# ultravideo/video-stitcher

Hardware: AMD Instinct MI355X
Metric: stitched frames/sec, 6x1080p->4K equirect (ms/frame = 1000/value*n_gpus) (higher is better)
Workload: dtype u8 in / int16+fp32 pyramid arithmetic; 1 GPU; cfg2: 6x1920x1080 views -> 3840x1920 equirect, spherical, 5 bands, CPW off; a step = 20 passes over a batch of 96 frames per GPU (1920 frames), each pass on 3 HIP stream(s) / contexts, inputs resident in HBM; distinct_frame_sets=8, frames_per_pass=96, streams=3, parallelism=frame-parallel x1

## Files before the change

video-stitcher_amd/csrc/compositor.hip:

```cpp
#include <algorithm>
#include <climits>
#include <memory>
#include <mutex>
#include <new>
#include <vector>
#include "common.hpp"
#include "launchers.hpp"
#include "descs.hpp"
#include "ctx.hpp"

namespace ms {

__device__ __forceinline__ void sample3(const uint8_t *__restrict__ src, unsigned sstep, int srows, int scols,
                                        float xc, float yc, float out[3])
{
    const int x1 = f2i_rd(xc), y1 = f2i_rd(yc);
    const int x2 = (int)((unsigned)x1 + 1u), y2 = (int)((unsigned)y1 + 1u);
    const float wx2 = (float)x2 - xc, wx1 = xc - (float)x1;
    const float wy2 = (float)y2 - yc, wy1 = yc - (float)y1;
    const float w[4] = {wx2 * wy2, wx1 * wy2, wx2 * wy1, wx1 * wy1};
    const int xs[4] = {x1, x2, x1, x2};
    const int ys[4] = {y1, y1, y2, y2};
    out[0] = out[1] = out[2] = 0.f;
#pragma unroll
    for (int t = 0; t < 4; ++t) {
        const bool inb = xs[t] >= 0 && xs[t] < scols && ys[t] >= 0 && ys[t] < srows;
        const uint8_t *p = src + (size_t)(inb ? ys[t] : 0) * sstep + (size_t)(inb ? xs[t] : 0) * 3;
#pragma unroll
        for (int c = 0; c < 3; ++c) out[c] = __builtin_fmaf(inb ? (float)p[c] : 0.f, w[t], out[c]);
    }
}

// ... 798 lines not shown
                } else {
                    const int k0 = (q >> 1) * 4 + (q & 1), k1 = k0 + 2;
                    DivBy d0(1.f), d1(1.f);
                    d0.d = den[r][k0]; d0.r = rcp[r][k0]; d1.d = den[r][k1]; d1.r = rcp[r][k1];
                    const int n0 = trunc_s16(d0((float)(int)(int16_t)(a & 0xffffu))), n1 = trunc_s16(d1((float)((int)a >> 16)));
                    n = ((unsigned)n0 & 0xffffu) | ((unsigned)n1 << 16);
                }
                resq[c][r][q] = addsat_pk_i16(upq[r][q], n);
            }
    }

    if (!L0) {
        const size_t plane = (size_t)P.qh[l] * P.qpitch[l];
        int16_t *d = cl + (size_t)f * cl_stride + P.coff[l] + (mul24(y0, P.qpitch[l]) + (unsigned)x0);
#pragma unroll
        for (int c = 0; c < 3; ++c)
#pragma unroll
            for (int r = 0; r < 2; ++r) {
                uint4 o;
                o.x = __builtin_amdgcn_perm(resq[c][r][1], resq[c][r][0], 0x05040100u);
                o.y = __builtin_amdgcn_perm(resq[c][r][1], resq[c][r][0], 0x07060302u);
                o.z = __builtin_amdgcn_perm(resq[c][r][3], resq[c][r][2], 0x05040100u);
                o.w = __builtin_amdgcn_perm(resq[c][r][3], resq[c][r][2], 0x07060302u);
                *reinterpret_cast<uint4 *>(d + c * plane + (size_t)r * P.qpitch[l]) = o;
            }
    } else {
#pragma unroll
        for (int r = 0; r < 2; ++r) {
            const int y = y0 + r;
            if (y >= P.fh) continue;
            const uint8_t *mrow = P.mask + mul24(y, P.mask_pitch);
            const int nvalid = min(8, P.fw - x0);
            uint2 mk8 = make_uint2(0u, 0u);
            if (nvalid == 8) __builtin_memcpy(&mk8, __builtin_assume_aligned(mrow + x0, 8), 8);
            else {
#pragma unroll
                for (int k = 0; k < 8; ++k) {
                    const unsigned m = (k < nvalid) ? (unsigned)mrow[x0 + k] : 0u;
                    if (k < 4) mk8.x |= m << (8 * k); else mk8.y |= m << (8 * (k - 4));
                }
            }
            const unsigned mq[4] = {__builtin_amdgcn_perm(0u, mk8.x, 0x02020000u), __builtin_amdgcn_perm(0u, mk8.x, 0x03030101u),
                                    __builtin_amdgcn_perm(0u, mk8.y, 0x02020000u), __builtin_amdgcn_perm(0u, mk8.y, 0x03030101u)};
            unsigned v[3][4];
#pragma unroll
            for (int c = 0; c < 3; ++c)
#pragma unroll
                for (int q = 0; q < 4; ++q) v[c][q] = resq[c][r][q] & mq[q];
            auto val = [&](int k, int c) -> int {
                const unsigned w = v[c][(k >> 2) * 2 + (k & 1)];
                return ((k >> 1) & 1) ? ((int)w >> 16) : (int)(int16_t)(w & 0xffffu);
            };
            if (out.p16[f]) {
                int16_t *d = (int16_t *)((char *)out.p16[f] + mul24(y, (int)out.step16[f])) + 3 * x0;
                if (nvalid == 8) {
                    unsigned wds[12];
#pragma unroll
// ... 492 lines not shown
            if (l >= 1) {
                const LevelDesc &F = V.lv[l - 1];
                Bits u = dilate(half(Wn[v][l - 1], F.w, F.h), L.w, L.h, 1);
                for (size_t i = 0; i < n.size(); ++i) n[i] |= u[i];
            }
            if (l < nb) {
                const LevelDesc &C = V.lv[l + 1];
                Bits d = dilate(twice(Nd[v][l + 1], C.w, C.h, L.w, L.h), L.w, L.h, 2);
                for (size_t i = 0; i < n.size(); ++i) n[i] |= d[i];
            }
            Nd[v][l] = std::move(n);
        }
        tot0 += (double)V.pw * V.ph;
    }
    c->warp_tiled = true;
    for (int v = 0; v < N; ++v) c->warp_tiled = c->warp_tiled && (c->h_views[v].pw % 4 == 0);
    c->warp_tiled = c->warp_tiled && c->cfg.src_width >= 3 && c->cfg.src_height >= 2;
    for (int v = 0; v < N; ++v) c->warp_tiled = c->warp_tiled && c->h_views[v].aw >= 3 && c->h_views[v].ah >= 2;
    {
        std::vector<WarpTile> tiles;
        for (int v = 0; v < N; ++v) {
            if (!((c->own_mask >> v) & 1u)) continue;
            const ViewDesc &V = c->h_views[v];
            for (int y0 = 0; y0 < V.ph; y0 += WARP_TH)
                for (int x0 = 0; x0 < V.pw; x0 += WARP_TW)
                    if (any_in(Nd[v][0], V.pw, V.ph, x0, y0, WARP_TW, WARP_TH)) {
                        WarpTile t{};
                        t.view = (short)v; t.x0 = (short)x0; t.y0 = (short)y0;
                        if (!c->custom_maps && x0 >= V.left && x0 + WARP_TW <= V.left + V.aw && y0 >= V.top && y0 + WARP_TH <= V.top + V.ah) {
                            t.flags |= 4;
                            t.ctab = (int)(c->tab_off[v] + (size_t)(x0 - V.left));
                            t.rtab = (int)(c->tab_off[v] + (size_t)round_up(V.aw, 4) + (size_t)(y0 - V.top));
                        }
                        tiles.push_back(t);
                        need0 += (double)std::min(WARP_TW, V.pw - x0) * std::min(WARP_TH, V.ph - y0);
                    }
        }
        c->needed_mask = 0;
        for (const WarpTile &t : tiles) c->needed_mask |= 1u << t.view;
        for (int v = 0; v < MAX_VIEWS; ++v) c->warp_per_view[v] = 0;
        for (const WarpTile &t : tiles) ++c->warp_per_view[t.view];
        if (!windowed || !c->warp_tiled) c->needed_mask = 0xffffffffu;
        if (c->cfg.raster_tile_order == 0) xcd_order(tiles, dev_knob("MS_XCD_CHUNK_WARP", c->cfg.enable_cpw ? 0 : 32));
        c->n_warp_tiles = (int)tiles.size();
        if (int e = c->warp_tiles.alloc(std::max<size_t>(1, tiles.size()) * sizeof(WarpTile))) return e;
        c->warp_lds_tiles = 0;
        if (!tiles.empty()) {
            MS_HIP(hipMemcpy(c->warp_tiles.p, tiles.data(), tiles.size() * sizeof(WarpTile), hipMemcpyHostToDevice));
            if (c->warp_tiled) {
                k_tile_bbox<<<c->n_warp_tiles, dim3(WARP_BX, std::min(WARP_TH, 256 / WARP_BX))>>>((WarpTile *)c->warp_tiles.p, (const ViewDesc *)c->view_tab.p, c->cfg.src_height, c->cfg.src_width, 0);
                MS_LAUNCH_CHECK();
                MS_HIP(hipMemcpy(tiles.data(), c->warp_tiles.p, tiles.size() * sizeof(WarpTile), hipMemcpyDeviceToHost));
                double sw_sum = 0; int sw_n = 0;
                for (const WarpTile &t : tiles) {
                    if (t.flags & 1) ++c->warp_lds_tiles;
                    if (t.sw > 0) { sw_sum += t.sw; ++sw_n; }
                }
                c->warp_minification = sw_n ? sw_sum / sw_n / WARP_TW : 0.0;
// ... 44 lines not shown
            for (const WarpTile &t : tiles) ((t.flags & 2) ? a : b).push_back(t);
            c->n_stage1_reachable = (int)a.size();
            if (c->cfg.raster_tile_order == 0) { xcd_order(a, dev_knob("MS_XCD_CHUNK_S1", 32)); xcd_order(b, dev_knob("MS_XCD_CHUNK_S1", 32)); }
            tiles = a;
            tiles.insert(tiles.end(), b.begin(), b.end());
        }
        c->n_stage1_tiles = (int)tiles.size();
        for (int v = 0; v < MAX_VIEWS; ++v) c->stage1_per_view[v] = 0;
        for (const WarpTile &t : tiles) ++c->stage1_per_view[t.view];
        if (int e = c->stage1_tiles.alloc(std::max<size_t>(1, tiles.size()) * sizeof(WarpTile))) return e;
        MS_HIP(hipMemcpy(c->stage1_tiles.p, tiles.data(), tiles.size() * sizeof(WarpTile), hipMemcpyHostToDevice));
        if (!tiles.empty() && c->warp_tiled) {
            k_tile_bbox<<<c->n_stage1_tiles, dim3(WARP_BX, std::min(WARP_TH, 256 / WARP_BX))>>>((WarpTile *)c->stage1_tiles.p, (const ViewDesc *)c->view_tab.p, c->cfg.src_height, c->cfg.src_width, 1);
            MS_LAUNCH_CHECK();
            MS_HIP(hipDeviceSynchronize());
        }
    }
    for (int l = 0; l < nb; ++l) {
        std::vector<DownTile> tiles;
        if (c->down_vec[l])
            for (int v = 0; v < N; ++v) {
                if (!((c->own_mask >> v) & 1u)) continue;
                const LevelDesc &Lo = c->h_views[v].lv[l + 1];
                for (int y0 = 0; y0 < Lo.h; y0 += DOWN_TH)
                    for (int x0 = 0; x0 < Lo.w; x0 += DOWN_TW)
                        if (any_in(Nd[v][l + 1], Lo.w, Lo.h, x0, y0, DOWN_TW, DOWN_TH)) tiles.push_back(DownTile{(short)v, 0, (short)x0, (short)y0});
            }
        if (c->cfg.raster_tile_order == 0) xcd_order(tiles, dev_knob(l == 0 ? "MS_XCD_CHUNK_DOWN0" : "MS_XCD_CHUNK_DOWN", 0));
        c->n_down_tiles[l] = (int)tiles.size();
        for (int v = 0; v < MAX_VIEWS; ++v) c->down_per_view[l][v] = 0;
        for (const DownTile &t : tiles) ++c->down_per_view[l][t.view];
        if (int e = c->down_tiles[l].alloc(std::max<size_t>(1, tiles.size()) * sizeof(DownTile))) return e;
        if (!tiles.empty()) MS_HIP(hipMemcpy(c->down_tiles[l].p, tiles.data(), tiles.size() * sizeof(DownTile), hipMemcpyHostToDevice));
    }
    for (int l = 0; l < nb; ++l) {
        std::vector<BlendTile> tiles;
        if (c->blend_vec[l])
            for (int y0 = 0; y0 < c->pano.qh[l]; y0 += BLEND_TH)
                for (int x0 = 0; x0 < c->pano.qw[l]; x0 += BLEND_TW) {
                    if (windowed && (x0 + BLEND_TW <= ra[l] || x0 >= rb[l])) continue;
                    unsigned m = 0;
                    for (int v = 0; v < N; ++v) {
                        const LevelDesc &L = c->h_views[v].lv[l];
                        if (any_in(W[v][l], L.w, L.h, x0 - L.x_tl, y0 - L.y_tl, BLEND_TW, BLEND_TH)) m |= 1u << v;
                    }
                    tiles.push_back(BlendTile{(short)x0, (short)y0, m});
                }
        if (c->cfg.raster_tile_order == 0) xcd_order(tiles, dev_knob(l == 0 ? "MS_XCD_CHUNK_BLEND0" : "MS_XCD_CHUNK_BLEND", (l == 0 && c->pano.qw[0] <= 4096) ? 8 : 0));
        c->n_blend_tiles[l] = (int)tiles.size();
// ... 468 lines not shown
}

static const uint8_t *blend_mask_ptr(const ms_ctx *c, int v)
{
    return (c->use_eff[v] ? (const uint8_t *)c->masks_eff.p : (const uint8_t *)c->masks.p) + c->mask_off[v];
}

int ms_init_blender(ms_ctx *c, ms_stream stream)
{
    if (!c) return fail(MS_ERR_INVALID, "null context");
    if (!c->maps_built || !c->masks_built) return fail(MS_ERR_STATE, "ms_init_blender: maps and masks must be built first");
    hipStream_t st = as_stream(stream);
    std::lock_guard<std::recursive_mutex> tables_lk(c->tables_mu);
    if (c->stitch_pending) MS_HIP(hipEventSynchronize(c->last_stitch));
    if (int e = pull_tracked_gains(c)) return e;
    const int nb = c->bg.num_bands, N = c->N, F = c->cfg.max_frames;
    c->act = nullptr; c->subset_on = false;
    ++c->tables_gen;
    if (c->subset_built_set) MS_HIP(hipEventSynchronize(c->subset_built));
    c->subsets.clear();
    c->zero_w.release();

    c->h_views.assign(N, ViewDesc{});
    size_t w_total = 0;
    long long g0_total = 64, gl_total = 64, stage_total = 0;
    c->max_pw = c->max_ph = c->max_aw = c->max_ah = 0;
    for (int v = 0; v < N; ++v) {
        ViewDesc &V = c->h_views[v];
        V.aw = c->roi[v].width; V.ah = c->roi[v].height;
        V.top = c->pad[v].top; V.left = c->pad[v].left;
        V.pw = V.aw + c->pad[v].left + c->pad[v].right;
        V.ph = V.ah + c->pad[v].top + c->pad[v].bottom;
        V.gain = (float)c->gain[v];
        V.xmap = (const float *)c->maps.p + c->map_off[v];
        V.ymap = V.xmap + (size_t)V.ah * c->map_pitch[v];
        V.map_pitch = c->map_pitch[v];
        if (c->custom_maps) V.proj = PROJ_MAPS;
        else {
            V.coltab = (const float2 *)c->tabs.p + c->tab_off[v];
            V.rowtab = V.coltab + round_up(V.aw, 4);
            V.wp = c->wparams[v];
            V.proj = c->cfg.projection;
        }
        V.s1_off = stage_total;
        V.s1_pitch = round_up(V.aw * 3, 4);
        stage_total += (long long)round_up(V.s1_pitch * V.ah + 8, 16);
        c->max_pw = std::max(c->max_pw, V.pw); c->max_ph = std::max(c->max_ph, V.ph);
        c->max_aw = std::max(c->max_aw, V.aw); c->max_ah = std::max(c->max_ah, V.ah);
        int w = V.pw, h = V.ph, xt = c->pad[v].x_tl, yt = c->pad[v].y_tl;
        for (int l = 0; l <= nb; ++l) {
            LevelDesc &L = V.lv[l];
            L.w = w; L.h = h; L.x_tl = xt; L.y_tl = yt;
            L.pitch = round_up(w, 16);
            L.wpitch = round_up(w, 4);
            c->w_off[v][l] = w_total;
            w_total += (size_t)h * L.wpitch;
            if (l == 0) { L.off = g0_total; g0_total += 3LL * h * L.pitch; }
            else        { L.off = gl_total; gl_total += 3LL * h * L.pitch; }
            w = (w + 1) / 2; h = (h + 1) / 2; xt /= 2; yt /= 2;
        }
    }
    for (int l = 0; l < nb; ++l) {
        bool ok = true;
        for (int v = 0; v < N; ++v) {
            const LevelDesc &L = c->h_views[v].lv[l];
            ok = ok && (L.w % 8 == 0) && (L.w >= 8) && (L.h >= 3);
        }
        c->down_vec[l] = ok;
    }
    {
        int t0 = 0;
        while (t0 < nb && c->down_vec[t0]) ++t0;
        auto plan_tail = [&](int l0, int sw, int *out_l0, int *out_lds, int *out_strips) {
            *out_l0 = -1; *out_lds = 0; *out_strips = 1;
            if (l0 < 1 || l0 >= nb) return;
            int need = 0, strips = 1;
            for (int v = 0; v < N; ++v) {
                int w[MAX_LEVELS + 1], a[MAX_LEVELS + 1], b[MAX_LEVELS + 1];
                for (int l = l0; l <= nb; ++l) w[l] = c->h_views[v].lv[l].w;
                const int ns = div_up(w[nb], sw);
                strips = std::max(strips, ns);
                for (int sidx = 0; sidx < ns; ++sidx) {
                    tail_range(w, l0, nb, sidx, sw, a, b);
                    int bytes = 0;
                    for (int l = l0; l <= nb; ++l) bytes += ((b[l] - a[l]) * c->h_views[v].lv[l].h + 15) & ~15;
                    need = std::max(need, bytes);
                }
            }
            if (need <= 64 * 1024) { *out_l0 = l0; *out_lds = need; *out_strips = strips; }
        };
        plan_tail(t0, TAIL_STRIP, &c->tail_l0, &c->tail_lds, &c->tail_strips);
        int l0b = -1;
        plan_tail(t0, TAIL_STRIP_BATCH, &l0b, &c->tail_lds_b, &c->tail_strips_b);
        if (l0b != c->tail_l0) { c->tail_lds_b = c->tail_lds; c->tail_strips_b = c->tail_strips; c->tail_sw_b = TAIL_STRIP; } else c->tail_sw_b = TAIL_STRIP_BATCH;
    }
    for (int l = 0; l < nb; ++l) {
        int qw = c->bg.dst_roi.width >> l, qh = c->bg.dst_roi.height >> l;
        bool ok = (qw % 8 == 0) && (qh % 2 == 0);
        for (int v = 0; v < N; ++v) {
            const LevelDesc &L = c->h_views[v].lv[l];
            ok = ok && (L.w % 8 == 0) && (L.x_tl % 8 == 0) && (L.h % 2 == 0) && (L.y_tl % 2 == 0);
        }
        c->blend_vec[l] = ok;
    }
    c->w_total = w_total;
    if (int e = c->weights.alloc(w_total * sizeof(float))) return e;
    MS_HIP(hipMemsetAsync(c->weights.p, 0, w_total * sizeof(float), st));
    {
        size_t m_total = 0;
        for (int v = 0; v < N; ++v) {
            ViewDesc &V = c->h_views[v];
            V.wm0_pitch = round_up(V.pw, 16);
            c->wm0_off[v] = m_total;
            m_total += (size_t)V.wm0_pitch * V.ph;
        }
        c->wm0_total = m_total + 64;
        if (int e = c->wm0.alloc(m_total + 64)) return e;
        MS_HIP(hipMemsetAsync(c->wm0.p, 0, m_total + 64, st));
        for (int v = 0; v < N; ++v) {
            ViewDesc &V = c->h_views[v];
            V.wm0 = (const uint8_t *)c->wm0.p + c->wm0_off[v];
            MS_HIP(hipMemcpy2DAsync((uint8_t *)c->wm0.p + c->wm0_off[v] + (size_t)V.top * V.wm0_pitch + V.left, V.wm0_pitch,
                                    blend_mask_ptr(c, v), V.aw, V.aw, V.ah, hipMemcpyDeviceToDevice, st));
        }
    }
    for (int v = 0; v < N; ++v)
        for (int l = 0; l <= nb; ++l) c->h_views[v].lv[l].wgt = (const float *)c->weights.p + c->w_off[v][l];

    PanoDesc &P = c->pano;
    P = PanoDesc{};
    P.nb = nb; P.n_views = N;
    size_t den_total = 0;
    long long cl_total = 32, pacc_total = 0;
    {
        int w = c->bg.dst_roi.width, h = c->bg.dst_roi.height;
        for (int l = 0; l <= nb; ++l) {
            P.qw[l] = w; P.qh[l] = h; P.qpitch[l] = round_up(w, 8); P.dpitch[l] = round_up(w, 4);
            c->den_off[l] = den_total; den_total += (size_t)h * P.dpitch[l];
            P.coff[l] = cl_total;
            if (l >= 1) cl_total += 3LL * h * P.qpitch[l];
            P.poff[l] = pacc_total;
            pacc_total += 3LL * h * P.qpitch[l];
            w = (w + 1) / 2; h = (h + 1) / 2;
        }
    }
    P.fw = c->bg.dst_roi_final.width; P.fh = c->bg.dst_roi_final.height;
    P.mask_pitch = round_up(P.fw, 16);
    P.alpha = (float)(1. / 255.);
    P.canvas_x = c->canvas_x; P.canvas_y = c->canvas_y; P.out_w = c->cfg.out_width; P.out_h = c->cfg.out_height;
    P.i_y0 = std::max(0, c->canvas_y & ~1); P.i_rows = std::max(0, std::min(c->cfg.out_height & ~1, (c->canvas_y + P.fh + 1) & ~1) - P.i_y0);
    c->den_total = den_total;
    if (int e = c->den.alloc(den_total * sizeof(float))) return e;
    if (int e = c->result_mask.alloc((size_t)P.mask_pitch * P.fh)) return e;
    MS_HIP(hipMemsetAsync(c->den.p, 0, den_total * sizeof(float), st));
    for (int l = 0; l <= nb; ++l) P.den[l] = (const float *)c->den.p + c->den_off[l];
    P.mask = (const uint8_t *)c->result_mask.p;
    {
        int t = 0;
        while (t < nb && c->blend_vec[t]) ++t;
        auto plan_btail = [&](int tt, int bw, int *out_t, int *out_lds, int *out_strips) {
            *out_t = -1; *out_lds = 0; *out_strips = 0;
            bool ok = tt >= 1 && tt < nb && c->cfg.debug_simple_kernels == 0;
            for (int l = tt; ok && l < nb; ++l) {
                ok = P.qw[l] % 2 == 0 && P.qh[l] % 2 == 0;
                for (int v = 0; ok && v < N; ++v) {
                    const LevelDesc &L = c->h_views[v].lv[l];
                    ok = L.w % 2 == 0 && L.h % 2 == 0 && L.x_tl % 2 == 0 && L.y_tl % 2 == 0;
                }
            }
            if (!ok) return;
// ... 1295 lines not shown
```

video-stitcher_amd/csrc/descs.hpp:

```cpp
#pragma once
#include "common.hpp"

namespace ms {

constexpr int MAX_LEVELS = 8;
constexpr int MAX_VIEWS = 16;
constexpr int MAX_SRC = 192;
constexpr int MAX_FRAMES = 64;
static_assert(MAX_SRC >= MAX_VIEWS, "a source table holds at least one frame of every view");
constexpr int PROJ_MAPS = 3;
static_assert(PROJ_MAPS != MS_PROJ_PLANE && PROJ_MAPS != MS_PROJ_CYLINDRICAL && PROJ_MAPS != MS_PROJ_SPHERICAL, "PROJ_MAPS must not name a projection");

struct LevelDesc {
    int w, h, pitch;
    int x_tl, y_tl;
    long long off;
    const float *wgt;
    int wpitch;
};
struct ViewDesc {
    int aw, ah;
    int top, left;
    int pw, ph;
    float gain;
    const float *xmap, *ymap;
    int map_pitch;
    const float2 *coltab, *rowtab;
    WarpParams wp;
    int proj;
    const uint8_t *wm0;
    int wm0_pitch;
    long long s1_off;
    int s1_pitch;
    LevelDesc lv[MAX_LEVELS];
};
struct PanoDesc {
    int nb, n_views;
    int qw[MAX_LEVELS], qh[MAX_LEVELS], qpitch[MAX_LEVELS];
// ... 7 lines not shown
    int fw, fh;
    int canvas_x, canvas_y, out_w, out_h;
    int i_y0, i_rows;
    const uint8_t *pure[MAX_LEVELS];
    int ppitch[MAX_LEVELS];
};
struct ShardArgs {
    int mode;
    unsigned own_mask;
    int n_parts;
    const int16_t *part[4];
    int16_t *pout;
    long long pstride;
};
struct SrcTable { const uint8_t *p[MAX_SRC]; unsigned step[MAX_SRC]; };
struct SrcAll { const uint8_t *p[MAX_FRAMES * MAX_VIEWS]; unsigned step[MAX_FRAMES * MAX_VIEWS]; };
struct MeshTable { const float *x[MAX_VIEWS]; const float *y[MAX_VIEWS]; int pitch[MAX_VIEWS]; };
struct DispTable { const unsigned *p[MAX_VIEWS]; unsigned limit_bits; };
struct OutTable { uint8_t *p8[MAX_FRAMES]; unsigned step8[MAX_FRAMES]; int16_t *p16[MAX_FRAMES]; unsigned step16[MAX_FRAMES];
                  uint8_t *pi[MAX_FRAMES]; };


struct WarpTile { short view, flags; short x0, y0; short sx0, sy0, sw, sh; int ctab, rtab; };
struct DownTile { short view, pad; short x0, y0; };
struct BlendTile { short x0, y0; unsigned view_mask; };

#ifndef MS_WARP_TW
#define MS_WARP_TW 32
#define MS_WARP_TH 16
#endif
constexpr int WARP_TW = MS_WARP_TW, WARP_TH = MS_WARP_TH;
constexpr int WARP_BX = WARP_TW / 4;
#ifndef MS_DOWN_ROWS
#define MS_DOWN_ROWS 4
#endif
constexpr int DOWN_ROWS = MS_DOWN_ROWS;
constexpr int DOWN_TW = 128, DOWN_TH = 8 * DOWN_ROWS;
constexpr int BLEND_TW = 256, BLEND_TH = 16;

}
```

video-stitcher_amd/csrc/tile_kernels.hpp:

```cpp
#pragma once
#include "descs.hpp"
#ifndef MS_PRIO_WARP
#define MS_PRIO_WARP 1
#endif
#ifndef MS_PRIO_CPW
#define MS_PRIO_CPW 0
#endif
#ifndef MS_PRIO_S1
#define MS_PRIO_S1 0
#endif
#ifndef MS_PRIO_NV12
#define MS_PRIO_NV12 0
#endif
#ifndef MS_PRIO_BLEND
#define MS_PRIO_BLEND 0
#endif
#define MS_PRIO_LOADS(K) do { if ((K) == 1 || (K) == 3) __builtin_amdgcn_s_setprio(3); else if ((K) == 2) __builtin_amdgcn_s_setprio(0); } while (0)
#define MS_PRIO_RELOADS(K) do { if ((K) == 1) __builtin_amdgcn_s_setprio(3); else if ((K) == 2) __builtin_amdgcn_s_setprio(0); } while (0)
#define MS_PRIO_MATH(K)  do { if ((K) == 1 || (K) == 3) __builtin_amdgcn_s_setprio(0); else if ((K) == 2) __builtin_amdgcn_s_setprio(3); } while (0)

namespace ms {

__device__ __forceinline__ int reflect_fast(int i, int len)
{
// ... 209 lines not shown
}

__device__ __forceinline__ void warp_coltab4(const ViewDesc &V, int x, float2 ct[4])
{
    const int i0 = x - V.left;
    if (i0 >= 0 && i0 + 3 < V.aw) {
        float4 a, b;
        a = gload_f4(V.coltab + i0);
        b = gload_f4(V.coltab + i0 + 2);
        ct[0] = make_float2(a.x, a.y); ct[1] = make_float2(a.z, a.w); ct[2] = make_float2(b.x, b.y); ct[3] = make_float2(b.z, b.w);
    } else {
#pragma unroll
        for (int k = 0; k < 4; ++k) ct[k] = gload_f2(V.coltab + reflect_fast(i0 + k, V.aw));
    }
}

__host__ __device__ __forceinline__ int warp_lds_ncopy(int sw) { return (3 * sw + 15 + 15) / 16; }
__host__ __device__ __forceinline__ int warp_lds_np(int sw) { return (warp_lds_ncopy(sw) + 1) | 1; }
#ifndef MS_WA_BUF
#define MS_WA_BUF 8192
#endif
constexpr int WA_BUF_BYTES = MS_WA_BUF;

__global__ void __launch_bounds__(256) k_tile_bbox(WarpTile *__restrict__ tiles, const ViewDesc *__restrict__ views, int src_rows, int src_cols, int stage1)
{
    __shared__ int s_box[5];
    WarpTile T = tiles[blockIdx.x];
    const ViewDesc &V = views[T.view];
    if (threadIdx.x == 0 && threadIdx.y == 0) { s_box[0] = s_box[2] = 0x7fffffff; s_box[1] = s_box[3] = -1; s_box[4] = -1; }
    __syncthreads();
    const int ox = stage1 ? V.left : 0, oy = stage1 ? V.top : 0;
    const int x = T.x0 + 4 * (int)threadIdx.x + ox;
    for (int y = T.y0 + (int)threadIdx.y + oy; y < T.y0 + oy + WARP_TH; y += (int)blockDim.y)
    if (stage1 ? (x - ox < V.aw && y - oy < V.ah) : (x < V.pw && y < V.ph)) {
        float xc[4], yc[4];
        MeshTable none{};
        if (V.proj == PROJ_MAPS) warp_coords4<false, PROJ_MAPS>(V, none, T.view, min(x, V.pw - 4), y, xc, yc);
        else warp_coords4<false>(V, none, T.view, min(x, V.pw - 4), y, xc, yc);
#pragma unroll
        for (int k = 0; k < 4; ++k) {
            const Taps t = make_taps(xc[k], yc[k], src_rows, src_cols);
            atomicMax(&s_box[4], min(max(f2i_rd(yc[k]), 0), src_rows - 2) + 1);
            if (t.fast) {
                atomicMin(&s_box[0], t.x1); atomicMax(&s_box[1], t.x1 + 1);
                atomicMin(&s_box[2], t.y1); atomicMax(&s_box[3], t.y1 + 1);
            }
        }
    }
    __syncthreads();
    if (threadIdx.x == 0 && threadIdx.y == 0) {
        T.flags &= ~(1 | 8);
        if (s_box[4] < src_rows - 1) T.flags |= 8;
        if (s_box[1] < 0) { T.sx0 = T.sy0 = T.sw = T.sh = 0; }
        else {
            const int sx0 = s_box[0] & ~3;
            const int sw = ((s_box[1] - sx0 + 1) + 3) & ~3, sh = s_box[3] - s_box[2] + 1;
            T.sx0 = (short)sx0; T.sy0 = (short)s_box[2]; T.sw = (short)sw; T.sh = (short)sh;
// ... 4 lines not shown
}

#ifndef MS_WARP_NG
#define MS_WARP_NG 1
#endif
constexpr int WARP_NG = MS_WARP_NG;
constexpr int WARP_BY = WARP_TH / WARP_NG;

#ifndef MS_WARP_NF_OPAQUE
#define MS_WARP_NF_OPAQUE 0
#endif
template <bool CPW, int PROJ, bool AL = false, int NF = 1, int NG = WARP_NG>
__device__ __forceinline__ void warp_tile_direct(const WarpTile &T, int f0, int nf, int tx, int ty, const ViewDesc *__restrict__ views, int n_views,
                                                 const SrcTable &src, int src_rows, int src_cols, const MeshTable &mesh,
                                                 const uint8_t *__restrict__ stage, long long stage_stride,
                                                 uint8_t *__restrict__ g0, long long g0_stride, const float2 *__restrict__ tabs)
{
    const int v = T.view;
    const ViewDesc &V = views[v];
    const int x = T.x0 + 4 * tx;
    int ys[NG];
    bool active[NG];
#pragma unroll
    for (int g = 0; g < NG; ++g) { ys[g] = T.y0 + ty + g * (WARP_TH / NG); active[g] = x < V.pw && ys[g] < V.ph; }
    const uint8_t *sp[NF];
    unsigned sstep[NF];
    int srows, scols;
#pragma unroll
    for (int fi = 0; fi < NF; ++fi) {
        const int f = f0 + (fi < nf ? fi : 0);
        if (CPW) { sp[fi] = stage + (size_t)f * stage_stride + V.s1_off; sstep[fi] = (unsigned)V.s1_pitch; }
        else { sp[fi] = src.p[f * n_views + v]; sstep[fi] = src.step[f * n_views + v]; }
    }
    if (CPW) { srows = V.ah; scols = V.aw; } else { srows = src_rows; scols = src_cols; }
    const LevelDesc &L = V.lv[0];
    const size_t plane = (size_t)L.h * L.pitch;
    float xc[2][4], yc[2][4];
    Px2 r1[2][4], r2[2][4];
    Px3 q1[AL ? 2 : 1][AL ? 4 : 1], q2[AL ? 2 : 1][AL ? 4 : 1];
    unsigned sh1[2] = {0u, 0u}, sh2[2] = {0u, 0u};
    constexpr bool DENSE = CPW || PROJ == PROJ_MAPS;
    float2 ct[4], rt[NG];
    if (!DENSE) {
        if (T.flags & 4) {
            float4 a, b;
            const float2 *cp = tabs + T.ctab + 4 * tx;
            __builtin_memcpy(&a, __builtin_assume_aligned(cp, 8), 16);
// ... 147 lines not shown
{
    const WarpTile T = tiles[blockIdx.x];
    constexpr int NF = warp_nf(CPW);
    const int f0 = (int)blockIdx.z * NF, nf = min(NF, n_frames - f0);
    if (AL && (CPW || (T.flags & 8)))
        warp_tile_direct<CPW, PROJ, true, NF>(T, f0, nf, (int)threadIdx.x, (int)(threadIdx.y + blockIdx.y * WARP_WY), views, n_views, src, src_rows, src_cols, mesh, stage, stage_stride,
                                                   g0, g0_stride, tabs);
    else
        warp_tile_direct<CPW, PROJ, false, NF>(T, f0, nf, (int)threadIdx.x, (int)(threadIdx.y + blockIdx.y * WARP_WY), views, n_views, src, src_rows, src_cols, mesh, stage, stage_stride,
                                                    g0, g0_stride, tabs);
}

template <bool CPW, int PROJ, int NF, bool AL = true>
__device__ __forceinline__ void warp_tile_shared(const WarpTile &T, int f0, int nf, int tx, int ty, const ViewDesc *__restrict__ views, int n_views,
                                                 const SrcTable &src, int src_rows, int src_cols, const MeshTable &mesh,
                                                 const uint8_t *__restrict__ stage, long long stage_stride,
                                                 uint8_t *__restrict__ g0, long long g0_stride, const float2 *__restrict__ tabs)
{
    constexpr int PRIO = CPW ? MS_PRIO_CPW : (AL ? MS_PRIO_WARP : 0);
    MS_PRIO_LOADS(PRIO);
    const int v = T.view;
    const ViewDesc &V = views[v];
    const int x = T.x0 + 4 * tx, y = T.y0 + ty;
    const bool active = x < V.pw && y < V.ph;
    ms_gptr_u8 base[NF];
    const uint8_t *ubase[NF];
    unsigned lo2 = 0u;
#pragma unroll
    for (int fi = 0; fi < NF; ++fi) {
        const int f = f0 + (fi < nf ? fi : 0);
        const uint8_t *p = CPW ? stage + (size_t)f * stage_stride + V.s1_off : src.p[f * n_views + v];
        base[fi] = (ms_gptr_u8)((uintptr_t)p & ~(uintptr_t)3);
        ubase[fi] = p;
        if (fi == 0 && AL) lo2 = (unsigned)(uintptr_t)p & 3u;
    }
    const unsigned st = CPW ? (unsigned)V.s1_pitch : src.step[f0 * n_views + v];
    const int srows = CPW ? V.ah : src_rows, scols = CPW ? V.aw : src_cols;
    const LevelDesc &L = V.lv[0];
    const size_t plane = (size_t)L.h * L.pitch;
    float xc[4], yc[4];
    if (CPW || PROJ == PROJ_MAPS) {
        if (active) warp_coords4<CPW, PROJ>(V, mesh, v, x, y, xc, yc);
    } else {
        float2 ct[4], rt;
        if (T.flags & 4) {
            float4 a, b;
            const float2 *cp = tabs + T.ctab + 4 * tx;
// ... 153 lines not shown
    }
}

constexpr int S1_BY_NV = WARP_TH;
typedef unsigned short ms_u16_a1 __attribute__((aligned(1)));
typedef unsigned ms_u32_a2 __attribute__((aligned(2)));
__device__ __forceinline__ NvRGB nv12_tap_checked(ms_gptr_u8 base, unsigned st, int rows, int cols, int xx, int yy)
{
    NvRGB z{0.f, 0.f, 0.f};
    if ((unsigned)xx >= (unsigned)cols || (unsigned)yy >= (unsigned)rows) return z;
    const unsigned Y = base[(unsigned)yy * st + (unsigned)xx];
    const unsigned o = (unsigned)(rows + (yy >> 1)) * st + (unsigned)(xx & ~1);
    return nv12_bgr(Y, (unsigned)base[o] | ((unsigned)base[o + 1] << 8));
}
template <int PROJ, int NF, bool ALN, bool S1>
__device__ __forceinline__ void nv12_tile(const WarpTile &T, int f0, int nf, int tx, int ty, const ViewDesc *__restrict__ views, int n_views,
                                          const SrcTable &src, int rows, int cols, uint8_t *__restrict__ g0, long long g0_stride, const float2 *__restrict__ tabs)
{
    constexpr int PRIO = S1 ? 0 : MS_PRIO_NV12;
    MS_PRIO_LOADS(PRIO);
    const int v = T.view;
    const ViewDesc &V = views[v];
    const int x = T.x0 + 4 * tx, y = T.y0 + ty;
    const bool active = S1 ? (x < V.aw && y < V.ah) : (x < V.pw && y < V.ph);
    if (S1 && !active) return;
    ms_gptr_u8 base[NF];
#pragma unroll
    for (int fi = 0; fi < NF; ++fi) base[fi] = (ms_gptr_u8)(uintptr_t)src.p[(f0 + (fi < nf ? fi : 0)) * n_views + v];
    const unsigned st = src.step[f0 * n_views + v];
    const LevelDesc &L = V.lv[0];
    const size_t plane = (size_t)L.h * L.pitch;
    float xc[4], yc[4];
    if (PROJ == PROJ_MAPS) {
        const MeshTable none{};
        if (active) warp_coords4<false, PROJ>(V, none, v, S1 ? x + V.left : x, S1 ? y + V.top : y, xc, yc);
        else {
#pragma unroll
            for (int k = 0; k < 4; ++k) xc[k] = yc[k] = -1.f;
        }
    } else {
        float2 ct[4], rt;
        if (S1) {
#pragma unroll
            for (int k = 0; k < 4; ++k) ct[k] = gload_f2(V.coltab + min(x + k, V.aw - 1));
            rt = gload_f2(V.rowtab + y);
        } else warp_tabs_load(T, views, tabs, tx, ty, ct, rt);
        if (active) {
// ... 211 lines not shown
#pragma unroll
            for (int k = 0; k < 4; ++k) ctn[k] = ct[k];
#pragma unroll
            for (int g = 0; g < WA_NG; ++g) rtn[g] = rt[g];
        }
        int tnn = tn, fnn = fn;
        advance(tnn, fnn);
        const WarpTile Tnn = tiles[fnn < n_frames ? tnn : t];
        if (!(T.flags & 1)) {
            warp_tile_direct<false, PROJ, false, 1, WA_NG>(T, f, 1, tx, ty, views, n_views, src, srows, scols, none, nullptr, 0, g0, g0_stride, tabs);
            __builtin_amdgcn_s_waitcnt(0x0F70);
        } else {
            const int v = T.view;
            const ViewDesc &V = views[v];
            const int x = T.x0 + 4 * tx;
            const uint8_t *sp = src.p[f * n_views + v];
            const unsigned sstep = src.step[f * n_views + v];
            const uint8_t *lb = lds + buf * WA_BUF_BYTES;
            const unsigned pitch = 16u * (unsigned)warp_lds_np(T.sw);
            const unsigned a0 = (unsigned)(((uintptr_t)sp + (size_t)T.sy0 * sstep + 3u * (unsigned)T.sx0) & 15u), astep = sstep & 15u;
            int ys[WA_NG];
            bool active[WA_NG];
#pragma unroll
            for (int g = 0; g < WA_NG; ++g) { ys[g] = T.y0 + ty + g * WA_BY; active[g] = x < V.pw && ys[g] < V.ph; }
            float xc[WA_NG][4], yc[WA_NG][4];
            Px2 r1[WA_NG][4], r2[WA_NG][4];
            bool slow = false;
#pragma unroll
            for (int g = 0; g < WA_NG; ++g)
#pragma unroll
                for (int k = 0; k < 4; ++k) {
                    if (active[g]) warp_combine(PROJ, ct[k], rt[g], V.wp, xc[g][k], yc[g][k]);
                    else xc[g][k] = yc[g][k] = -1.f;
                    const int x1 = f2i_rd(xc[g][k]), y1 = f2i_rd(yc[g][k]);
                    const bool fast = (unsigned)x1 < (unsigned)(scols - 2) && (unsigned)y1 < (unsigned)(srows - 1);
                    slow = slow || (active[g] && !fast);
                    const int lx = min(max(x1 - (int)T.sx0, 0), (int)T.sw - 2), ly = min(max(y1 - (int)T.sy0, 0), (int)T.sh - 2);
                    const unsigned o1 = (unsigned)ly * pitch + ((a0 + (unsigned)ly * astep) & 15u) + 3u * (unsigned)lx;
                    const unsigned o2 = (unsigned)(ly + 1) * pitch + ((a0 + (unsigned)(ly + 1) * astep) & 15u) + 3u * (unsigned)lx;
                    r1[g][k] = lds_px2(lb, o1);
                    r2[g][k] = lds_px2(lb, o2);
                }
            if (__builtin_amdgcn_ballot_w64(slow)) {
#pragma unroll
                for (int g = 0; g < WA_NG; ++g)
#pragma unroll
                    for (int k = 0; k < 4; ++k) {
// ... 296 lines not shown
}
__device__ __forceinline__ unsigned down_hpass(const Down7 &v)
{
    const unsigned e01 = __builtin_amdgcn_alignbyte(v.a[1], v.a[0], 2), e12 = v.a[1], e23 = __builtin_amdgcn_alignbyte(v.a[2], v.a[1], 2);
    const unsigned e34 = v.a[2], e45 = __builtin_amdgcn_alignbyte(v.a[3], v.a[2], 2);
    const unsigned o01 = __builtin_amdgcn_alignbyte(v.a[5], v.a[4], 2), o12 = v.a[5], o23 = __builtin_amdgcn_alignbyte(v.a[6], v.a[5], 2), o34 = v.a[6];
    const unsigned s01 = mad6(e12, e01 + e23 + 4u * (o01 + o12));
    const unsigned s23 = mad6(e34, e23 + e45 + 4u * (o23 + o34));
    return __builtin_amdgcn_perm(rne8_pk(s23), rne8_pk(s01), 0x06040200u);
}

template <bool L0>
__global__ void __launch_bounds__(256) __attribute__((amdgpu_waves_per_eu(6, 8))) k_down_t(const DownTile *__restrict__ tiles, const ViewDesc *__restrict__ views, int l,
                                                const uint8_t *__restrict__ gin, long long in_stride,
                                                uint8_t *__restrict__ gout, long long out_stride)
{
    const DownTile T = tiles[blockIdx.x];
    const int c = blockIdx.y, f = blockIdx.z, v = T.view;
    const int ty = (int)threadIdx.y;
    const LevelDesc &Li = views[v].lv[l], &Lo = views[v].lv[l + 1];
    constexpr int RO = DOWN_ROWS, RI = 2 * RO + 3;
    const int t = (T.x0 >> 2) + (int)threadIdx.x;
    const int y = T.y0 + RO * ty;
    if (4 * t >= Lo.w || y >= Lo.h) return;
    const uint8_t *in = gin + (size_t)f * in_stride + Li.off + (size_t)c * Li.h * Li.pitch;
    const int nrow = min(RO, Lo.h - y);
    const int sy = 2 * y, last = Li.h - 1;
    int ridx[RI];
    ridx[0] = abs(sy - 2); ridx[1] = abs(sy - 1); ridx[2] = sy;
#pragma unroll
    for (int j = 3; j < RI; ++j) { const int r = sy + j - 2; ridx[j] = r > last ? 2 * last - r : r; }
#pragma unroll
    for (int j = 5; j < RI; ++j) if (j > 2 * nrow + 2) ridx[j] = ridx[4];
    Row11u8 raw[RI];
#pragma unroll
    for (int j = 0; j < RI; ++j) raw[j] = fetch_row11(in + (size_t)ridx[j] * Li.pitch, t, Li.w);
    Down7 r[RI];
#pragma unroll
    for (int j = 0; j < RI; ++j) r[j] = down_row(raw[j], t, Li.w);
    uint8_t *out = gout + (size_t)f * out_stride + Lo.off + (size_t)c * Lo.h * Lo.pitch + (size_t)y * Lo.pitch + 4 * t;
#pragma unroll
    for (int o = 0; o < RO; ++o) {
        Down7 vv;
#pragma unroll
        for (int k = 0; k < 7; ++k) vv.a[k] = mad6(r[2 * o + 2].a[k], (r[2 * o].a[k] + r[2 * o + 4].a[k]) + 4u * (r[2 * o + 1].a[k] + r[2 * o + 3].a[k]));
        if (o < nrow) *reinterpret_cast<unsigned *>(out + (size_t)o * Lo.pitch) = down_hpass(vv);
    }
// ... 4 lines not shown
```

Before: 36450 frames/s.

## Anchor pyramid planes to 128-byte lines and align tile grids to them

Adds a line_layout helper that places view, weight, mask and panorama planes so that pixels at pano-aligned x land on 128-byte line boundaries via a per-plane lead offset. Warp and down tile grids get a narrow first tile so later tiles start on line boundaries, with lanes of the narrow tile masked through new flag bits and DownTile width. It also skips the L0 mask load for pure tiles. The aim is fewer partially touched cache lines per tile access, at the cost of extra padding, more tiles and one extra per-lane predicate.

```diff
diff --git a/video-stitcher_amd/csrc/compositor.hip b/video-stitcher_amd/csrc/compositor.hip
--- a/video-stitcher_amd/csrc/compositor.hip
+++ b/video-stitcher_amd/csrc/compositor.hip
@@ -8,6 +8,26 @@
 #include "launchers.hpp"
 #include "descs.hpp"
 #include "ctx.hpp"
+#include "line_layout.hpp"
+#ifndef MS_LAYOUT_COLL_LEAD
+#define MS_LAYOUT_COLL_LEAD 0
+#endif
+#ifndef MS_LAYOUT_VIEW_SHIFT
+#define MS_LAYOUT_VIEW_SHIFT 0
+#endif
+#ifndef MS_L0_MASK_SKIP
+#define MS_L0_MASK_SKIP 1
+#endif
+#ifndef MS_WARP_ANCHOR
+#define MS_WARP_ANCHOR 1
+#endif
+#ifndef MS_DOWN_ANCHOR
+#define MS_DOWN_ANCHOR 1
+#endif
+#ifndef MS_DOWN_PHASE
+#define MS_DOWN_PHASE 4
+#endif
+static_assert(MS_DOWN_PHASE % 4 == 0 && MS_DOWN_PHASE >= 0 && MS_DOWN_PHASE < 128, "reduce tiles start on a 4-pixel strip");
 
 namespace ms {
 
@@ -852,7 +872,7 @@
                 o.y = __builtin_amdgcn_perm(resq[c][r][1], resq[c][r][0], 0x07060302u);
                 o.z = __builtin_amdgcn_perm(resq[c][r][3], resq[c][r][2], 0x05040100u);
                 o.w = __builtin_amdgcn_perm(resq[c][r][3], resq[c][r][2], 0x07060302u);
-                *reinterpret_cast<uint4 *>(d + c * plane + (size_t)r * P.qpitch[l]) = o;
+                __builtin_memcpy(__builtin_assume_aligned(d + c * plane + (size_t)r * P.qpitch[l], MS_LAYOUT_COLL_LEAD % 8 == 0 ? 16 : 4), &o, 16);
             }
     } else {
 #pragma unroll
@@ -862,7 +882,8 @@
             const uint8_t *mrow = P.mask + mul24(y, P.mask_pitch);
             const int nvalid = min(8, P.fw - x0);
             uint2 mk8 = make_uint2(0u, 0u);
-            if (nvalid == 8) __builtin_memcpy(&mk8, __builtin_assume_aligned(mrow + x0, 8), 8);
+            if (MS_L0_MASK_SKIP && pure && nvalid == 8) mk8 = make_uint2(0xffffffffu, 0xffffffffu);
+            else if (nvalid == 8) __builtin_memcpy(&mk8, __builtin_assume_aligned(mrow + x0, 8), 8);
             else {
 #pragma unroll
                 for (int k = 0; k < 8; ++k) {
@@ -1401,18 +1422,20 @@
         for (int v = 0; v < N; ++v) {
             if (!((c->own_mask >> v) & 1u)) continue;
             const ViewDesc &V = c->h_views[v];
+            const int first = MS_WARP_ANCHOR ? (WARP_TW - V.lv[0].lead % WARP_TW) % WARP_TW : 0;
             for (int y0 = 0; y0 < V.ph; y0 += WARP_TH)
-                for (int x0 = 0; x0 < V.pw; x0 += WARP_TW)
-                    if (any_in(Nd[v][0], V.pw, V.ph, x0, y0, WARP_TW, WARP_TH)) {
+                for (int x0 = 0, tw = first ? first : WARP_TW; x0 < V.pw; x0 += tw, tw = WARP_TW)
+                    if (any_in(Nd[v][0], V.pw, V.ph, x0, y0, tw, WARP_TH)) {
                         WarpTile t{};
                         t.view = (short)v; t.x0 = (short)x0; t.y0 = (short)y0;
+                        if (tw < WARP_TW) t.flags |= (short)((tw / 4) << 4);
                         if (!c->custom_maps && x0 >= V.left && x0 + WARP_TW <= V.left + V.aw && y0 >= V.top && y0 + WARP_TH <= V.top + V.ah) {
                             t.flags |= 4;
                             t.ctab = (int)(c->tab_off[v] + (size_t)(x0 - V.left));
                             t.rtab = (int)(c->tab_off[v] + (size_t)round_up(V.aw, 4) + (size_t)(y0 - V.top));
                         }
                         tiles.push_back(t);
-                        need0 += (double)std::min(WARP_TW, V.pw - x0) * std::min(WARP_TH, V.ph - y0);
+                        need0 += (double)std::min(tw, V.pw - x0) * std::min(WARP_TH, V.ph - y0);
                     }
         }
         c->needed_mask = 0;
@@ -1503,9 +1526,10 @@
             for (int v = 0; v < N; ++v) {
                 if (!((c->own_mask >> v) & 1u)) continue;
                 const LevelDesc &Lo = c->h_views[v].lv[l + 1];
+                const int first = MS_DOWN_ANCHOR ? (DOWN_TW + MS_DOWN_PHASE - Lo.lead % DOWN_TW) % DOWN_TW : 0;
                 for (int y0 = 0; y0 < Lo.h; y0 += DOWN_TH)
-                    for (int x0 = 0; x0 < Lo.w; x0 += DOWN_TW)
-                        if (any_in(Nd[v][l + 1], Lo.w, Lo.h, x0, y0, DOWN_TW, DOWN_TH)) tiles.push_back(DownTile{(short)v, 0, (short)x0, (short)y0});
+                    for (int x0 = 0, tw = first ? first : DOWN_TW; x0 < Lo.w; x0 += tw, tw = DOWN_TW)
+                        if (any_in(Nd[v][l + 1], Lo.w, Lo.h, x0, y0, tw, DOWN_TH)) tiles.push_back(DownTile{(short)v, (short)tw, (short)x0, (short)y0});
             }
         if (c->cfg.raster_tile_order == 0) xcd_order(tiles, dev_knob(l == 0 ? "MS_XCD_CHUNK_DOWN0" : "MS_XCD_CHUNK_DOWN", 0));
         c->n_down_tiles[l] = (int)tiles.size();
@@ -2020,8 +2044,7 @@
     c->zero_w.release();
 
     c->h_views.assign(N, ViewDesc{});
-    size_t w_total = 0;
-    long long g0_total = 64, gl_total = 64, stage_total = 0;
+    long long stage_total = 0;
     c->max_pw = c->max_ph = c->max_aw = c->max_ah = 0;
     for (int v = 0; v < N; ++v) {
         ViewDesc &V = c->h_views[v];
@@ -2049,12 +2072,6 @@
         for (int l = 0; l <= nb; ++l) {
             LevelDesc &L = V.lv[l];
             L.w = w; L.h = h; L.x_tl = xt; L.y_tl = yt;
-            L.pitch = round_up(w, 16);
-            L.wpitch = round_up(w, 4);
-            c->w_off[v][l] = w_total;
-            w_total += (size_t)h * L.wpitch;
-            if (l == 0) { L.off = g0_total; g0_total += 3LL * h * L.pitch; }
-            else        { L.off = gl_total; gl_total += 3LL * h * L.pitch; }
             w = (w + 1) / 2; h = (h + 1) / 2; xt /= 2; yt /= 2;
         }
     }
@@ -2101,20 +2118,39 @@
         }
         c->blend_vec[l] = ok;
     }
+    LineLayoutIn lin;
+    lin.n_views = N; lin.nb = nb;
+    lin.lv.resize((size_t)N * (nb + 1)); lin.view_anchored.assign(nb + 1, 0); lin.pano_anchored.assign(nb + 1, 0);
+    for (int v = 0; v < N; ++v)
+        for (int l = 0; l <= nb; ++l) { const LevelDesc &L = c->h_views[v].lv[l]; lin.lv[(size_t)v * (nb + 1) + l] = LayoutLevel{L.w, L.h, L.x_tl}; }
+    for (int l = 0; l < nb; ++l) {
+        lin.view_anchored[l] = c->cfg.debug_simple_kernels == 0 && (c->down_vec[l] || c->blend_vec[l]);
+        lin.pano_anchored[l] = c->cfg.debug_simple_kernels == 0 && c->blend_vec[l];
+    }
+    lin.pano_w = c->bg.dst_roi.width; lin.pano_h = c->bg.dst_roi.height; lin.final_w = c->bg.dst_roi_final.width;
+    lin.coll_lead = MS_LAYOUT_COLL_LEAD; lin.view_shift = MS_LAYOUT_VIEW_SHIFT;
+    const LineLayout lay = line_layout(lin);
+    for (int v = 0; v < N; ++v)
+        for (int l = 0; l <= nb; ++l) {
+            LevelDesc &L = c->h_views[v].lv[l];
+            const PlaneSpot &s = lay.view[(size_t)v * (nb + 1) + l], &ws = lay.wgt[(size_t)v * (nb + 1) + l];
+            L.pitch = s.pitch; L.off = s.off; L.lead = s.lead;
+            L.wpitch = ws.pitch; c->w_off[v][l] = (size_t)ws.off;
+        }
+    const size_t w_total = (size_t)lay.w_total;
+    const long long g0_total = lay.g0_total, gl_total = lay.gl_total;
     c->w_total = w_total;
     if (int e = c->weights.alloc(w_total * sizeof(float))) return e;
     MS_HIP(hipMemsetAsync(c->weights.p, 0, w_total * sizeof(float), st));
     {
-        size_t m_total = 0;
         for (int v = 0; v < N; ++v) {
             ViewDesc &V = c->h_views[v];
-            V.wm0_pitch = round_up(V.pw, 16);
-            c->wm0_off[v] = m_total;
-            m_total += (size_t)V.wm0_pitch * V.ph;
-        }
-        c->wm0_total = m_total + 64;
-        if (int e = c->wm0.alloc(m_total + 64)) return e;
-        MS_HIP(hipMemsetAsync(c->wm0.p, 0, m_total + 64, st));
+            V.wm0_pitch = lay.wm0[v].pitch;
+            c->wm0_off[v] = (size_t)lay.wm0[v].off;
+        }
+        c->wm0_total = (size_t)lay.wm0_total;
+        if (int e = c->wm0.alloc(c->wm0_total)) return e;
+        MS_HIP(hipMemsetAsync(c->wm0.p, 0, c->wm0_total, st));
         for (int v = 0; v < N; ++v) {
             ViewDesc &V = c->h_views[v];
             V.wm0 = (const uint8_t *)c->wm0.p + c->wm0_off[v];
@@ -2128,22 +2164,20 @@
     PanoDesc &P = c->pano;
     P = PanoDesc{};
     P.nb = nb; P.n_views = N;
-    size_t den_total = 0;
-    long long cl_total = 32, pacc_total = 0;
+    const size_t den_total = (size_t)lay.den_total;
+    const long long cl_total = lay.cl_total, pacc_total = lay.pacc_total;
     {
         int w = c->bg.dst_roi.width, h = c->bg.dst_roi.height;
         for (int l = 0; l <= nb; ++l) {
-            P.qw[l] = w; P.qh[l] = h; P.qpitch[l] = round_up(w, 8); P.dpitch[l] = round_up(w, 4);
-            c->den_off[l] = den_total; den_total += (size_t)h * P.dpitch[l];
-            P.coff[l] = cl_total;
-            if (l >= 1) cl_total += 3LL * h * P.qpitch[l];
-            P.poff[l] = pacc_total;
-            pacc_total += 3LL * h * P.qpitch[l];
+            P.qw[l] = w; P.qh[l] = h; P.qpitch[l] = lay.qpitch[l]; P.dpitch[l] = lay.den[l].pitch;
+            c->den_off[l] = (size_t)lay.den[l].off;
+            P.coff[l] = lay.coll[l].off;
+            P.poff[l] = lay.part[l].off;
             w = (w + 1) / 2; h = (h + 1) / 2;
         }
     }
     P.fw = c->bg.dst_roi_final.width; P.fh = c->bg.dst_roi_final.height;
-    P.mask_pitch = round_up(P.fw, 16);
+    P.mask_pitch = lay.mask_pitch;
     P.alpha = (float)(1. / 255.);
     P.canvas_x = c->canvas_x; P.canvas_y = c->canvas_y; P.out_w = c->cfg.out_width; P.out_h = c->cfg.out_height;
     P.i_y0 = std::max(0, c->canvas_y & ~1); P.i_rows = std::max(0, std::min(c->cfg.out_height & ~1, (c->canvas_y + P.fh + 1) & ~1) - P.i_y0);
diff --git a/video-stitcher_amd/csrc/descs.hpp b/video-stitcher_amd/csrc/descs.hpp
--- a/video-stitcher_amd/csrc/descs.hpp
+++ b/video-stitcher_amd/csrc/descs.hpp
@@ -14,6 +14,7 @@
 struct LevelDesc {
     int w, h, pitch;
     int x_tl, y_tl;
+    int lead;
     long long off;
     const float *wgt;
     int wpitch;
@@ -67,7 +68,7 @@
 
 
 struct WarpTile { short view, flags; short x0, y0; short sx0, sy0, sw, sh; int ctab, rtab; };
-struct DownTile { short view, pad; short x0, y0; };
+struct DownTile { short view, w; short x0, y0; };
 struct BlendTile { short x0, y0; unsigned view_mask; };
 
 #ifndef MS_WARP_TW
@@ -76,6 +77,7 @@
 #endif
 constexpr int WARP_TW = MS_WARP_TW, WARP_TH = MS_WARP_TH;
 constexpr int WARP_BX = WARP_TW / 4;
+static_assert(WARP_BX <= 16 && WARP_TW % 4 == 0, "WarpTile::flags bits 4-7 hold the lanes of a narrow first tile");
 #ifndef MS_DOWN_ROWS
 #define MS_DOWN_ROWS 4
 #endif
diff --git a/video-stitcher_amd/csrc/line_layout.hpp b/video-stitcher_amd/csrc/line_layout.hpp
--- /dev/null
+++ b/video-stitcher_amd/csrc/line_layout.hpp
@@ -0,0 +1,93 @@
+#pragma once
+#include <vector>
+
+namespace ms {
+
+constexpr int LINE_BYTES = 128;
+
+struct LayoutLevel { int w, h, x_tl; };
+struct PlaneSpot { long long off; int pitch, lead; };
+
+struct LineLayoutIn {
+    int n_views = 0, nb = 0;
+    std::vector<LayoutLevel> lv;
+    std::vector<char> view_anchored;
+    int pano_w = 0, pano_h = 0;
+    std::vector<char> pano_anchored;
+    int final_w = 0;
+    int coll_lead = 0;
+    int view_shift = 0;
+};
+struct LineLayout {
+    std::vector<PlaneSpot> view;
+    long long g0_total = 0, gl_total = 0;
+    std::vector<PlaneSpot> coll, part;
+    std::vector<int> qpitch;
+    long long cl_total = 0, pacc_total = 0;
+    std::vector<PlaneSpot> wgt;
+    long long w_total = 0;
+    std::vector<PlaneSpot> den;
+    long long den_total = 0;
+    std::vector<PlaneSpot> wm0;
+    long long wm0_total = 0;
+    int mask_pitch = 0;
+};
+
+inline long long layout_round_up(long long a, long long m) { return (a + m - 1) / m * m; }
+
+inline PlaneSpot layout_place(long long &total, int w, int h, int planes, int esz, bool anchored, int lead, int compact_align)
+{
+    const int line = LINE_BYTES / esz;
+    PlaneSpot s{};
+    if (anchored) {
+        total = layout_round_up(total, line);
+        s.lead = lead; s.pitch = (int)layout_round_up((long long)lead + w, line); s.off = total + lead;
+        total += (long long)planes * h * s.pitch;
+    } else {
+        s.lead = 0; s.pitch = (int)layout_round_up(w, compact_align); s.off = total;
+        total += (long long)planes * h * s.pitch;
+    }
+    return s;
+}
+
+inline LineLayout line_layout(const LineLayoutIn &in)
+{
+    const int N = in.n_views, nl = in.nb + 1;
+    LineLayout o;
+    o.view.resize((size_t)N * nl); o.wgt.resize((size_t)N * nl); o.wm0.resize(N);
+    o.coll.resize(nl); o.part.resize(nl); o.den.resize(nl); o.qpitch.resize(nl);
+    auto lead_of = [](int x_tl, int esz, int need) { return (x_tl % need == 0 && x_tl >= 0) ? (int)(((long long)x_tl * esz) % LINE_BYTES) / esz : 0; };
+    o.g0_total = o.gl_total = LINE_BYTES;
+    for (int v = 0; v < N; ++v)
+        for (int l = 0; l < nl; ++l) {
+            const LayoutLevel &L = in.lv[(size_t)v * nl + l];
+            const bool a = in.view_anchored[l] != 0;
+            int lead = lead_of(L.x_tl, 1, 4);
+            if (l >= 1 && L.x_tl % 4 == 0 && L.x_tl >= 0) lead = (lead + in.view_shift) % LINE_BYTES;
+            o.view[(size_t)v * nl + l] = layout_place(l == 0 ? o.g0_total : o.gl_total, L.w, L.h, 3, 1, a, lead, 16);
+            o.wgt[(size_t)v * nl + l] = layout_place(o.w_total, L.w, L.h, 1, 4, a && l < in.nb && in.pano_anchored[l], lead_of(L.x_tl, 4, 4), 4);
+            if (l == 0) o.wm0[v] = layout_place(o.wm0_total, L.w, L.h, 1, 1, a && in.pano_anchored[0], lead_of(L.x_tl, 1, 8), 16);
+        }
+    o.g0_total = layout_round_up(o.g0_total, LINE_BYTES); o.gl_total = layout_round_up(o.gl_total, LINE_BYTES);
+    o.w_total = layout_round_up(o.w_total, LINE_BYTES / 4);
+    o.wm0_total = layout_round_up(o.wm0_total, LINE_BYTES) + 64;
+    o.cl_total = LINE_BYTES / 2;
+    int w = in.pano_w, h = in.pano_h;
+    for (int l = 0; l < nl; ++l) {
+        const bool a = in.pano_anchored[l] != 0;
+        o.part[l] = layout_place(o.pacc_total, w + (a ? in.coll_lead : 0), h, 3, 2, a, 0, 8);
+        o.qpitch[l] = o.part[l].pitch;
+        if (l >= 1) {
+            if (a) o.cl_total = layout_round_up(o.cl_total, LINE_BYTES / 2);
+            o.coll[l] = PlaneSpot{o.cl_total + (a ? in.coll_lead : 0), o.qpitch[l], a ? in.coll_lead : 0};
+            o.cl_total += 3LL * h * o.qpitch[l];
+        } else o.coll[l] = PlaneSpot{o.cl_total, o.qpitch[l], 0};
+        o.den[l] = layout_place(o.den_total, w, h, 1, 4, a, 0, 4);
+        w = (w + 1) / 2; h = (h + 1) / 2;
+    }
+    o.cl_total = layout_round_up(o.cl_total, LINE_BYTES / 2); o.pacc_total = layout_round_up(o.pacc_total, LINE_BYTES / 2);
+    o.mask_pitch = (int)layout_round_up(in.final_w, in.pano_anchored[0] ? LINE_BYTES : 16);
+    return o;
+}
+
+}
diff --git a/video-stitcher_amd/csrc/tile_kernels.hpp b/video-stitcher_amd/csrc/tile_kernels.hpp
--- a/video-stitcher_amd/csrc/tile_kernels.hpp
+++ b/video-stitcher_amd/csrc/tile_kernels.hpp
@@ -255,6 +255,12 @@
 #endif
 constexpr int WA_BUF_BYTES = MS_WA_BUF;
 
+__device__ __forceinline__ bool warp_lane_in(const WarpTile &T, int tx)
+{
+    const int n = (T.flags >> 4) & 15;
+    return n == 0 || tx < n;
+}
+
 __global__ void __launch_bounds__(256) k_tile_bbox(WarpTile *__restrict__ tiles, const ViewDesc *__restrict__ views, int src_rows, int src_cols, int stage1)
 {
     __shared__ int s_box[5];
@@ -265,7 +271,7 @@
     const int ox = stage1 ? V.left : 0, oy = stage1 ? V.top : 0;
     const int x = T.x0 + 4 * (int)threadIdx.x + ox;
     for (int y = T.y0 + (int)threadIdx.y + oy; y < T.y0 + oy + WARP_TH; y += (int)blockDim.y)
-    if (stage1 ? (x - ox < V.aw && y - oy < V.ah) : (x < V.pw && y < V.ph)) {
+    if (stage1 ? (x - ox < V.aw && y - oy < V.ah) : (x < V.pw && y < V.ph && warp_lane_in(T, (int)threadIdx.x))) {
         float xc[4], yc[4];
         MeshTable none{};
         if (V.proj == PROJ_MAPS) warp_coords4<false, PROJ_MAPS>(V, none, T.view, min(x, V.pw - 4), y, xc, yc);
@@ -316,7 +322,7 @@
     int ys[NG];
     bool active[NG];
 #pragma unroll
-    for (int g = 0; g < NG; ++g) { ys[g] = T.y0 + ty + g * (WARP_TH / NG); active[g] = x < V.pw && ys[g] < V.ph; }
+    for (int g = 0; g < NG; ++g) { ys[g] = T.y0 + ty + g * (WARP_TH / NG); active[g] = x < V.pw && ys[g] < V.ph && warp_lane_in(T, tx); }
     const uint8_t *sp[NF];
     unsigned sstep[NF];
     int srows, scols;
@@ -510,7 +516,7 @@
     const int v = T.view;
     const ViewDesc &V = views[v];
     const int x = T.x0 + 4 * tx, y = T.y0 + ty;
-    const bool active = x < V.pw && y < V.ph;
+    const bool active = x < V.pw && y < V.ph && warp_lane_in(T, tx);
     ms_gptr_u8 base[NF];
     const uint8_t *ubase[NF];
     unsigned lo2 = 0u;
@@ -710,7 +716,7 @@
     const int v = T.view;
     const ViewDesc &V = views[v];
     const int x = T.x0 + 4 * tx, y = T.y0 + ty;
-    const bool active = S1 ? (x < V.aw && y < V.ah) : (x < V.pw && y < V.ph);
+    const bool active = S1 ? (x < V.aw && y < V.ah) : (x < V.pw && y < V.ph && warp_lane_in(T, tx));
     if (S1 && !active) return;
     ms_gptr_u8 base[NF];
 #pragma unroll
@@ -968,7 +974,7 @@
             int ys[WA_NG];
             bool active[WA_NG];
 #pragma unroll
-            for (int g = 0; g < WA_NG; ++g) { ys[g] = T.y0 + ty + g * WA_BY; active[g] = x < V.pw && ys[g] < V.ph; }
+            for (int g = 0; g < WA_NG; ++g) { ys[g] = T.y0 + ty + g * WA_BY; active[g] = x < V.pw && ys[g] < V.ph && warp_lane_in(T, tx); }
             float xc[WA_NG][4], yc[WA_NG][4];
             Px2 r1[WA_NG][4], r2[WA_NG][4];
             bool slow = false;
@@ -1311,7 +1317,7 @@
     constexpr int RO = DOWN_ROWS, RI = 2 * RO + 3;
     const int t = (T.x0 >> 2) + (int)threadIdx.x;
     const int y = T.y0 + RO * ty;
-    if (4 * t >= Lo.w || y >= Lo.h) return;
+    if (4 * (int)threadIdx.x >= T.w || 4 * t >= Lo.w || y >= Lo.h) return;
     const uint8_t *in = gin + (size_t)f * in_stride + Li.off + (size_t)c * Li.h * Li.pitch;
     const int nrow = min(RO, Lo.h - y);
     const int sy = 2 * y, last = Li.h - 1;
```

Result: faster. 37310 frames/s, median of 6 (+2.3%).
